# sevagh/demucs.cpp

Measured on AMD Instinct MI355X. Metric: audio-sec/s (xRT) htdemucs-4s 44.1kHz stereo, ~4-min track with overlap-add (BASELINE configs[2]), higher is better.
Workload: dtype f32 (exact bf16x3 operand split, fp32 accumulate)

## Files before the change

demucs_cpp_amd/binding.py:

```python
from __future__ import annotations

import ctypes
import os
from typing import List, Optional, Tuple

import numpy as np

ROOT = os.path.dirname(os.path.dirname(os.path.abspath(__file__)))
LIB_PATH = os.environ.get("DMX_LIB", os.path.join(ROOT, "demucs_cpp_amd", "lib", "libdemucs_hip.so"))

LAYOUT_EIGEN = 0
LAYOUT_PLANAR = 1
SEGMENT_SAMPLES = 343980
MAX_SHIFT = 22050
MAX_BAG = 8

EXPORTS = [
    "dmx_last_error", "dmx_device_count", "dmx_model_load", "dmx_model_free", "dmx_model_n_sources",
    "dmx_model_n_tensors", "dmx_model_device", "dmx_ctx_create", "dmx_ctx_free", "dmx_ctx_segment_samples",
    "dmx_ctx_max_batch", "dmx_ctx_arena_bytes", "dmx_ctx_synchronize", "dmx_ctx_set_stream", "dmx_segment_infer",
    "dmx_segment_infer_device", "dmx_track_infer", "dmx_track_geometry", "dmx_track_stats_device",
    "dmx_track_gather_device", "dmx_track_overlap_add_device", "dmx_debug_tap", "dmx_debug_n_ops",
    "dmx_debug_profile", "dmx_ctx_set_model", "dmx_model_clone",
    "dmx_debug_plan_info", "dmx_debug_op_info", "dmx_debug_arena_fill", "dmx_debug_arena_io", "dmx_debug_run_op", "dmx_debug_op_cfgs",
# ... 104 lines not shown
        L.dmx_remix_two_stems.argtypes = [ci, ci, ci, vp, vp]
        L.dmx_remix_check.argtypes = [ci, vp]
        L.dmx_tracks_infer_remix.argtypes = [vp, vp, ci, vp, ci, vp, vp, ci, ctypes.c_float, vp, vp, vp, vp, ci, vp, vp]
        L.dmx_remix_encode_device.argtypes = [ci, vp, ci, i64, i64, vp, vp, vp, vp, vp]
        L.dmx_remix_encode.argtypes = [ci, vp, ci, i64, vp, vp, vp, vp]
        L.dmx_flac_bound.argtypes = [ci, i64]
        L.dmx_flac_bound.restype = i64
        L.dmx_flac_workspace_bytes.argtypes = [ci, i64]
        L.dmx_flac_workspace_bytes.restype = i64
        L.dmx_flac_encode_device.argtypes = [ci, vp, ci, i64, ci, vp, vp, vp, vp]
        L.dmx_flac_encode.argtypes = [ci, vp, ci, i64, ci, vp, vp]
        L.dmx_tracks_infer_flac.argtypes = [vp, vp, ci, vp, ci, vp, vp, ci, ctypes.c_float, vp, vp, ci, vp, vp, vp, ci, vp, vp]
        L.dmx_track_geometry.argtypes = [vp, i64, ci, ctypes.POINTER(i64), ctypes.POINTER(ci), ctypes.POINTER(i64)]
        L.dmx_track_stats_device.argtypes = [vp, fp, i64, fp]
        L.dmx_track_gather_device.argtypes = [vp, fp, i64, fp, ci, vp, ci, fp]
        L.dmx_track_overlap_add_device.argtypes = [vp, fp, ci, i64, ci, fp, fp, ci]
        L.dmx_debug_tap.argtypes = [vp, ctypes.c_char_p, vp, fp]
        L.dmx_debug_n_ops.argtypes = [vp]
        L.dmx_debug_profile.argtypes = [vp, ci, ci, ctypes.c_char_p, ci]
        L.dmx_debug_plan_info.argtypes = [vp, ci, vp, vp, vp, vp]
        L.dmx_debug_op_info.argtypes = [vp, ci, ci, ctypes.c_char_p, ci]
        L.dmx_debug_arena_fill.argtypes = [vp, ci, ctypes.c_uint]
        L.dmx_debug_arena_io.argtypes = [vp, i64, i64, fp, ci]
        L.dmx_debug_run_op.argtypes = [vp, ci, ci]
        L.dmx_debug_op_cfgs.argtypes = [vp, ci, ci, vp, ci]
        L.dmx_debug_run_op_as.argtypes = [vp, ci, ci, ci, ci, ctypes.c_char_p, ci]
        L.dmx_ctx_set_model.argtypes = [vp, vp]
        L.dmx_engine_create.argtypes = [ctypes.POINTER(ctypes.c_char_p), ci, ctypes.POINTER(ci), ci, ci, ci, ctypes.POINTER(vp)]
        L.dmx_engine_free.argtypes = [vp]
        L.dmx_engine_set_finish.argtypes = [vp, ci]
        for f in ("dmx_engine_n_devices", "dmx_engine_n_models", "dmx_engine_n_sources", "dmx_engine_transport", "dmx_engine_finish"):
            getattr(L, f).argtypes = [vp]
        L.dmx_engine_root_ctx.argtypes = [vp, ci]
        L.dmx_engine_root_ctx.restype = vp
        L.dmx_engine_track_infer.argtypes = [vp, fp, i64, ctypes.POINTER(ci), fp, ci, vp, vp]
        _lib = L
    return _lib


def _chk(rc):
    if rc != 0:
        raise DmxError(rc, lib().dmx_last_error().decode(errors="replace"))


DEBUG_NO_KERNEL = 6


def parse_op_info(text: str) -> dict:
    d = {}
    for word in text.split():
        k, _, v = word.partition("=")
        if k in ("reads", "writes", "scratch", "rowstat"):
            d[k] = [tuple(int(x) for x in r.split(":")) for r in v.split(",") if r]
        elif k in ("name", "label"):
            d[k] = v
        else:
            d[k] = int(v)
    return d


def device_count() -> int:
    return lib().dmx_device_count()


class Model:

    def __init__(self, path: str, device: int = 0):
        self.h = ctypes.c_void_p()
        _chk(lib().dmx_model_load(path.encode(), device, ctypes.byref(self.h)))
        self.n_sources = lib().dmx_model_n_sources(self.h)
        self.n_tensors = lib().dmx_model_n_tensors(self.h)
        self.arch = lib().dmx_model_arch(self.h)
        self.device = device

    def close(self):
        if self.h:
            lib().dmx_model_free(self.h)
            self.h = ctypes.c_void_p()

    def __del__(self):
        try:
            self.close()
        except Exception:
            pass


def default_gemm() -> int:
    return lib().dmx_default_gemm()


def set_default_gemm(gemm: int):
    _chk(lib().dmx_set_default_gemm(gemm))


def split_weights(w: np.ndarray):
    w = np.ascontiguousarray(w, np.float32).ravel()
    w1 = np.zeros(w.size, np.uint16)
    w2 = np.zeros(w.size, np.uint16)
    bad = lib().dmx_debug_split_weights(w.ctypes.data, w.size, w1.ctypes.data, w2.ctypes.data)
    return w1, w2, int(bad)


def split_activations(x: np.ndarray, device: int = 0) -> np.ndarray:
    x = np.ascontiguousarray(x, np.float32).ravel()
    planes = np.zeros((3, x.size), np.uint16)
    _chk(lib().dmx_debug_split_activations(device, x.ctypes.data, x.size, planes.ctypes.data))
    return planes
# ... 574 lines not shown
```

demucs_cpp_amd/csrc/api.cpp:

```cpp
#include "api_internal.h"
#include "tracks_plan.h"
#include "plan_describe.h"

#include <algorithm>
#include <atomic>
#include <cstdarg>
#include <cstdio>
#include <cstdlib>
#include <cmath>
#include <cstring>
#include <cctype>
#include <cerrno>
#include <climits>
#include <fcntl.h>
#include <pthread.h>
#include <signal.h>
#include <sys/mman.h>
#include <sys/stat.h>
#include <unistd.h>

using namespace dmx;

static thread_local std::string g_err;
int dmx_fail(int code, const char *fmt, ...)
// ... 245 lines not shown
            (void)hipFree(m->dWh);
    }
    delete m;
}
extern "C" int dmx_model_n_sources(const dmx_model *m) { return m ? m->pm.n_sources : 0; }
extern "C" int dmx_model_n_tensors(const dmx_model *m) { return m ? m->pm.n_tensors : 0; }
extern "C" int dmx_model_device(const dmx_model *m) { return m ? m->device : -1; }
extern "C" int dmx_model_arch(const dmx_model *m) { return m ? m->pm.arch : 0; }

static bool validate_gemm(const Op &op, std::string &why)
{
    const IGemm &g = op.g;
    const bool al = ((i64)g.L0 * g.Cin) % 4 == 0 && (g.stride0 * g.Cin) % 4 == 0 && (g.pad0 * g.Cin) % 4 == 0 &&
                    g.seg0 % 4 == 0 && g.K % 4 == 0 && g.xBatchStride % 4 == 0 && (g.S1 == 1 || g.seg0 % 16 == 0) &&
                    (g.cfg == kDirectCfg || (g.Cin % 4 == 0 && g.seg0 % g.Cin == 0 && g.S1 * (g.seg0 / g.Cin) <= 31));
    if (g.epi == EPI_KPL || g.epi == EPI_VT)
    {
        if (g.choice.arith == 0)
        {
            why = "op " + op.name + ": K / V plane projection without its exact-split kernel";
            return false;
        }
        return true;
    }
    GemmArgs k{};
    fill_gemm_geometry(k, g);
    const bool exists = (g.cfg == kDirectCfg ? launch_dgemm(k, nullptr, true) : launch_igemm(g.cfg, k, nullptr, true)) == 0;
    if (!al || !exists)
    {
        why = "op " + op.name + (al ? ": no kernel instantiated for its (tile, prologue, epilogue)" : ": staging alignment contract violated");
        return false;
    }
    return true;
}
static bool validate_plan(const Plan &p, std::string &why)
{
    for (const Op &op : p.ops)
        if (op.kind == OP_IGEMM && !validate_gemm(op, why))
            return false;
    return true;
}

static Plan *get_plan(dmx_ctx *c, int batch)
{
    auto it = c->plans.find(batch);
    if (it != c->plans.end())
        return it->second.get();
    auto p = std::make_unique<Plan>();
    const bool planesOff = getenv("DMX_KV_PLANES") && atoi(getenv("DMX_KV_PLANES")) == 0;
    AttnArgs kv{};
    kv.hs = c->m->pm.dim / 8;
    const bool kvPlanes = c->gemm != DMX_GEMM_F32 && !planesOff && c->m->pm.arch != 3 && launch_attention_split(kv, nullptr, true) == 0;
    build_chosen_plan(c->m->pm, c->seg, batch, c->gemm, kvPlanes, model_facts(c->m), split_lin_mode(), *p);
    for (Op &op : p->ops)
        if (op.kind == OP_ATTENTION)
        {
            AttnArgs t{};
            t.hs = op.at.hs;
            op.at.split = c->gemm != DMX_GEMM_F32 && launch_attention_split(t, nullptr, true) == 0 ? 1 : 0;
        }
    Plan *raw = p.get();
    c->plans[batch] = std::move(p);
    return raw;
}

struct SharedLane
{
    static const int kSlots = 64;
    std::atomic<int> ready;
    std::atomic<int> pid[kSlots];
    pthread_mutex_t mu;
};
struct LstmLane
{
    std::mutex mu;
    hipEvent_t ev = nullptr;
    bool recorded = false;
    SharedLane *shared = nullptr;
};
static std::mutex g_lanesMu;
static std::vector<std::unique_ptr<LstmLane>> g_lanes;
static std::vector<SharedLane *> g_sharedRegistered;

static bool pid_alive(int pid) { return pid > 0 && (kill((pid_t)pid, 0) == 0 || errno != ESRCH); }

static int shared_lane_peers(SharedLane *sl)
{
    const int self = (int)getpid();
    int n = 0;
    for (int i = 0; i < SharedLane::kSlots; ++i)
    {
        int p = sl->pid[i].load(std::memory_order_acquire);
        if (p == 0 || p == self)
            continue;
        if (pid_alive(p))
            ++n;
        else
            sl->pid[i].compare_exchange_strong(p, 0);
    }
    return n;
}

static SharedLane *open_shared_lane(int device)
{
    if (const char *e = getenv("DMX_LSTM_SHARED_LANE"))
        if (atoi(e) == 0)
            return nullptr;
    auto give_up = [](const char *what) -> SharedLane * {
        fprintf(stderr, "demucs_hip: the process-shared LSTM lane is unavailable (%s: %s); several Demucs v3 processes on one GPU are not ordered\n", what,
                strerror(errno));
        return nullptr;
    };
// ... 406 lines not shown
            k.Wb2 = c->m->dWb + c->m->blobFloats + 512 + g.w_w;
            rc = launch_igemm_split(g.choice, g.cfg, k, s);
            break;
        }
        if (rc != 0)
            return fail(DMX_ERR_ARG, "internal error: the kernel chosen for op %s does not exist (%s: family %d, cfg %d pro %d epi %d)", op.name.c_str(),
                        g.choice.label ? g.choice.label : "none", g.choice.family, g.cfg, g.pro, g.epi);
        break;
    }
    case OP_DCONV_ROW:
    {
        const DconvRow &r = op.dr;
        DconvRowArgs k{};
        k.x = a(r.x), k.B = r.B, k.T = r.T, k.F = r.F, k.C = r.C, k.hid = r.hid, k.eps = r.eps, k.zero = A + zeroOff;
        k.img[0] = w(r.img_w[0]), k.img[1] = w(r.img_w[1]);
        if (launch_dconv_row(k, s) != 0)
            return fail(DMX_ERR_ARG, "internal error: no row-resident DConv kernel for op %s (C %d hidden %d T %d)", op.name.c_str(), r.C, r.hid, r.T);
        break;
    }
    case OP_STATS_REDUCE:
    {
        const StatsReduce &r = op.sr;
        launch_stats_reduce(ReduceArgs{a(r.rowstat), a(r.out), r.B, r.R, r.NB, r.G0, r.count, r.mode, r.eps,
                                       reinterpret_cast<double *>(a(r.scratch)), r.nchunk},
                            s);
        break;
    }
    case OP_STFT:
    {
        const Stft &t = op.stft;
        launch_stft(StftArgs{a(t.mix), a(t.x), a(t.rowstat), a(t.rowstatT), t.B, t.T, t.seg, t.pad, a(t.window), a(t.twiddle)}, s);
        break;
    }
    case OP_LAYERNORM:
    {
        const LayerNorm &l = op.ln;
        launch_layernorm(LnArgs{a(l.x), a(l.y), l.rows, l.D, l.rowsPerBatch, w(l.w_w), w(l.b_w), a(l.pe), l.eps}, s);
        break;
    }
    case OP_GN_APPLY:
    {
        const GnApply &g = op.gn;
        launch_gn_apply(GnArgs{a(g.x), a(g.y), a(g.res), g.B, g.rows, g.C, a(g.stats), w(g.w_w), w(g.b_w)}, s);
        break;
    }
    case OP_ATTENTION:
    {
        const Attention &t = op.at;
        AttnArgs k{a(t.q), a(t.k), a(t.v), a(t.o), t.ldq, t.ldk, t.ldv, t.ldo, t.qBatch, t.kBatch, t.vBatch,
                   t.oBatch, t.B, t.Tq, t.Tk, t.H, t.hs, t.scale};
        k.kpl = t.kpl >= 0 ? reinterpret_cast<const unsigned short *>(A + t.kpl) : nullptr;
        k.vt = t.vt >= 0 ? reinterpret_cast<const unsigned short *>(A + t.vt) : nullptr;
        k.kvPlane = (i64)t.B * t.Tk * t.H * t.hs;
        if (!(t.split && launch_attention_split(k, s) == 0))
        {
            if (t.kpl >= 0)
                return fail(DMX_ERR_ARG, "internal error: attention op %s reads operand planes but has no exact-split kernel", op.name.c_str());
            launch_attention(k, s);
        }
        break;
    }
    case OP_ISTFT:
    {
        const Istft &t = op.istft;
        if (!(t.fused && c->fuseIstft))
            launch_istft(IstftArgs{a(t.x), a(t.stats), a(t.frames), t.B, t.T, t.S, a(t.window), a(t.twiddle)}, s);
        break;
    }
    case OP_OLA:
    {
        const Ola &o = op.ola;
        if (o.x >= 0 && c->fuseIstft)
            launch_istft_ola(IstftOlaArgs{a(o.x), a(o.stats), a(o.xt), a(o.statsT), a(o.wss), a(o.window), a(o.twiddle), a(o.out), o.B, o.T,
                                          o.S, o.seg, o.pad, 0, 0, a(o.rden)},
                             s);
        else
            launch_ola(OlaArgs{a(o.frames), a(o.xt), a(o.statsT), a(o.wss), a(o.out), o.B, o.T, o.S, o.seg, o.pad}, s);
        break;
    }
    case OP_GROUP_STATS:
    {
        const GroupStats &g = op.gs;
        launch_group_stats(GroupStatsArgs{a(g.x), a(g.out), reinterpret_cast<double *>(a(g.scratch)), g.B, g.rows, g.C, g.G, g.eps}, s);
        break;
    }
    case OP_GN_ACT:
    {
        const GnAct &g = op.ga;
        launch_gn_act(GnActArgs{a(g.x), a(g.y), a(g.stats), a(g.res), w(g.w_w), w(g.b_w), w(g.scale_w), g.B, g.rowsIn, g.C, g.G, g.mode,
                                g.rowOff, g.rowsOut},
                      s);
        break;
    }
    case OP_LSTM:
    {
        const Lstm &l = op.lstm;
        LstmLane *lane = c->capturing ? nullptr : lstm_lane(c->m->device);
        std::unique_lock<std::mutex> laneLock;
        if (lane)
        {
            laneLock = std::unique_lock<std::mutex>(lane->mu);
            if (!lane->ev)
                HIPCHK(hipEventCreateWithFlags(&lane->ev, hipEventDisableTiming));
            if (lane->recorded)
                HIPCHK(hipStreamWaitEvent(s, lane->ev, 0));
        }
// ... 1681 lines not shown
```

demucs_cpp_amd/csrc/attention_common.h:

```cpp
#pragma once
#include "kernels.h"

namespace dmx
{

typedef float f32x4 __attribute__((ext_vector_type(4)));

__device__ __forceinline__ float max3f(float a, float b, float c) { return __builtin_fmaxf(__builtin_fmaxf(a, b), c); }
static constexpr float kDeferLog2 = 16.0f;
static constexpr float kLog2e = 1.44269504088896340736f;

__device__ __forceinline__ float quad_lanes_max(float x)
{
    typedef unsigned u32x2 __attribute__((ext_vector_type(2)));
    u32x2 r = __builtin_amdgcn_permlane16_swap(__float_as_uint(x), __float_as_uint(x), false, false);
    x = fmaxf(__uint_as_float(r[0]), __uint_as_float(r[1]));
    r = __builtin_amdgcn_permlane32_swap(__float_as_uint(x), __float_as_uint(x), false, false);
    return fmaxf(__uint_as_float(r[0]), __uint_as_float(r[1]));
}
__device__ __forceinline__ float quad_lanes_sum(float x)
{
    typedef unsigned u32x2 __attribute__((ext_vector_type(2)));
    u32x2 r = __builtin_amdgcn_permlane16_swap(__float_as_uint(x), __float_as_uint(x), false, false);
    x = __uint_as_float(r[0]) + __uint_as_float(r[1]);
    r = __builtin_amdgcn_permlane32_swap(__float_as_uint(x), __float_as_uint(x), false, false);
    return __uint_as_float(r[0]) + __uint_as_float(r[1]);
}

template <int DF, bool MASK, bool LOC>
__device__ __forceinline__ void att_softmax_pre(f32x4 (&sT)[4], f32x4 (&o)[DF], float &mrun, float &lrun, float &mcur, int t, int h4, int Tk,
                                                int qrow, float gq)
{
    constexpr int KT = 64;
    if constexpr (LOC)
    {
#pragma unroll
        for (int kf = 0; kf < 4; ++kf)
#pragma unroll
            for (int r = 0; r < 4; ++r)
            {
                const int key = t * KT + 16 * kf + 4 * h4 + r;
                const float dist = fabsf((float)(key - qrow));
                sT[kf][r] = key == qrow ? -100.0f * kLog2e : sT[kf][r] - dist * gq;
            }
    }
    if constexpr (MASK)
    {
#pragma unroll
        for (int kf = 0; kf < 4; ++kf)
#pragma unroll
            for (int r = 0; r < 4; ++r)
                if (t * KT + 16 * kf + 4 * h4 + r >= Tk)
                    sT[kf][r] = -INFINITY;
// ... 4 lines not shown
    tmx2 = max3f(tmx2, sT[2][0], sT[2][1]);
    float tmx3 = max3f(sT[2][2], sT[2][3], sT[3][0]);
    tmx3 = max3f(tmx3, sT[3][1], sT[3][2]);
    tmax = max3f(tmax, tmx2, fmaxf(tmx3, sT[3][3]));
    tmax = quad_lanes_max(tmax);
    float mnew = mrun;
    if (__builtin_amdgcn_ballot_w64(tmax > mnew + kDeferLog2) != 0ull)
    {
        mnew = fmaxf(mnew, tmax);
        const float alpha = __builtin_amdgcn_exp2f(mrun - mnew);
        lrun *= alpha;
        mrun = mnew;
#pragma unroll
        for (int d = 0; d < DF; ++d)
        {
            o[d][0] *= alpha;
            o[d][1] *= alpha;
            o[d][2] *= alpha;
            o[d][3] *= alpha;
        }
    }
    mcur = mnew;
}
__device__ __forceinline__ void att_softmax_post(f32x4 (&sT)[4], float &lrun, float mcur)
{
    float ps[4] = {0.f, 0.f, 0.f, 0.f};
#pragma unroll
    for (int kf = 0; kf < 4; ++kf)
#pragma unroll
        for (int r = 0; r < 4; ++r)
        {
            const float pv = __builtin_amdgcn_exp2f(sT[kf][r] - mcur);
            sT[kf][r] = pv;
            ps[kf] += pv;
        }
    lrun += (ps[0] + ps[1]) + (ps[2] + ps[3]);
}

__device__ __forceinline__ bool att_tile_of_block(const AttnArgs &p, unsigned &qt, unsigned &bh)
{
    if (p.xcdMap)
    {
        const unsigned xcd = blockIdx.x & 7u, j = blockIdx.x >> 3;
        const unsigned g = j / p.nQt;
        qt = j - g * p.nQt;
        bh = g * 8u + xcd;
        return bh < (unsigned)(p.B * p.H);
    }
    bh = blockIdx.x / p.nQt;
    qt = blockIdx.x - bh * p.nQt;
    return true;
}

inline bool att_use_big_shape(const AttnArgs &a)
{
    const long wg128 = (long)((a.Tq + 127) / 128) * a.H * a.B, wg64 = (long)((a.Tq + 63) / 64) * a.H * a.B;
    const double costBig = (double)((wg128 + 511) / 512), costSmall = 0.6 * (double)((wg64 + 511) / 512);
    return wg128 >= 1024 && costBig <= costSmall;
}

}
```

demucs_cpp_amd/csrc/attention_split.hip:

```cpp
#include "attention_common.h"
#include "igemm_common.h"
#include <cstdlib>
#include <type_traits>

namespace dmx
{

__device__ __forceinline__ int swzK(int key) { return (key >> 1) & 7; }
__device__ __forceinline__ int swzV(int dim) { return ((dim >> 1) & 1) | (((dim >> 3) & 1) << 1) | (((dim >> 2) & 1) << 2); }

template <int HS, int QF, bool PL>
__global__ __launch_bounds__(256, 2) void attention_split_kernel(const AttnArgs p)
{
    constexpr int DF = HS / 16;
    constexpr int KT = 64;
    constexpr int NS = 8;
    constexpr int KSL = HS / 8;
    constexpr int KCH = (KT * KSL + 255) / 256;
    constexpr int DQ = HS / 4;
    static_assert(HS == 64 || HS == 48, "head dims of htdemucs (512 / 8, 384 / 8)");

    __shared__ u32x4 Kp0[3][KT][NS], Kp1[3][KT][NS];
    __shared__ u32x4 Vp[3][HS][NS];

    const int tid = threadIdx.x, lane = tid & 63, wave = tid >> 6;
    const int l15 = lane & 15, h4 = lane >> 4;
    unsigned qt, bh;
    if (!att_tile_of_block(p, qt, bh))
        return;
    const int b = (int)(bh / (unsigned)p.H), head = (int)(bh - (unsigned)b * (unsigned)p.H);
    const int q0 = (int)qt * (64 * QF) + wave * (16 * QF);
    const float *Q = p.q + (i64)b * p.qB + head * HS;
    const float *K = p.k + (i64)b * p.kB + head * HS;
    const float *V = p.v + (i64)b * p.vB + head * HS;

    if constexpr (KSL < NS)
    {
        for (int i = tid; i < 2 * 3 * KT * (NS - KSL); i += 256)
        {
            const int sl = KSL + i % (NS - KSL), key = (i / (NS - KSL)) % KT, pl = (i / ((NS - KSL) * KT)) % 3, bf = i / ((NS - KSL) * KT * 3);
            (bf ? Kp1 : Kp0)[pl][key][sl ^ swzK(key)] = u32x4{0u, 0u, 0u, 0u};
        }
    }

    const float qs = p.scale * kLog2e;
    u32x4 qp[3][QF][2];
#pragma unroll
    for (int f = 0; f < QF; ++f)
    {
        const int qr = min(q0 + 16 * f + l15, p.Tq - 1);
#pragma unroll
        for (int kk = 0; kk < 2; ++kk)
        {
            const int d0 = 32 * kk + 8 * h4;
            f32x4 v0 = f32x4{0.f, 0.f, 0.f, 0.f}, v1 = v0;
            if (d0 < HS)
            {
                v0 = *reinterpret_cast<const f32x4 *>(Q + (i64)qr * p.ldq + d0);
                v1 = *reinterpret_cast<const f32x4 *>(Q + (i64)qr * p.ldq + d0 + 4);
            }
            unsigned h1[4], h2[4], h3[4];
            split3_pk(v0[0] * qs, v0[1] * qs, h1[0], h2[0], h3[0]);
            split3_pk(v0[2] * qs, v0[3] * qs, h1[1], h2[1], h3[1]);
            split3_pk(v1[0] * qs, v1[1] * qs, h1[2], h2[2], h3[2]);
            split3_pk(v1[2] * qs, v1[3] * qs, h1[3], h2[3], h3[3]);
            qp[0][f][kk] = u32x4{h1[0], h1[1], h1[2], h1[3]};
            qp[1][f][kk] = u32x4{h2[0], h2[1], h2[2], h2[3]};
            qp[2][f][kk] = u32x4{h3[0], h3[1], h3[2], h3[3]};
        }
    }

    f32x4 kreg[KCH][2], vreg[4];
    const int vh4 = tid & 3, vhalf = (tid >> 2) & 1, vdq = ((tid >> 3) & 1) + 2 * ((tid >> 4) & 7), vs = tid >> 7;
    const int vkq4 = 8 * vs + 4 * vhalf + vh4;
    const bool vOk = vdq < DQ;
    auto load_k = [&](int t0) {
#pragma unroll
        for (int i = 0; i < KCH; ++i)
        {
            const int c = min(tid + 256 * i, KT * KSL - 1);
            const int key = c / KSL, sl = c - key * KSL;
            const i64 r = min(t0 + key, p.Tk - 1);
            kreg[i][0] = *reinterpret_cast<const f32x4 *>(K + r * p.ldk + 8 * sl);
            kreg[i][1] = *reinterpret_cast<const f32x4 *>(K + r * p.ldk + 8 * sl + 4);
        }
    };
    auto load_v = [&](int t0) {
#pragma unroll
        for (int j = 0; j < 4; ++j)
        {
            const i64 r = min(t0 + 4 * vkq4 + j, p.Tk - 1);
            vreg[j] = *reinterpret_cast<const f32x4 *>(V + r * p.ldv + 4 * (vOk ? vdq : 0));
        }
    };
    auto store_k = [&](int buf) {
#pragma unroll
        for (int i = 0; i < KCH; ++i)
        {
            const int c = tid + 256 * i;
            if (KT * KSL % 256 != 0 && c >= KT * KSL)
                continue;
            const int key = c / KSL, sl = c - key * KSL;
            unsigned h1[4], h2[4], h3[4];
            split3_pk(kreg[i][0][0], kreg[i][0][1], h1[0], h2[0], h3[0]);
            split3_pk(kreg[i][0][2], kreg[i][0][3], h1[1], h2[1], h3[1]);
            split3_pk(kreg[i][1][0], kreg[i][1][1], h1[2], h2[2], h3[2]);
            split3_pk(kreg[i][1][2], kreg[i][1][3], h1[3], h2[3], h3[3]);
            u32x4(*Kp)[KT][NS] = buf ? Kp1 : Kp0;
            const int sw = sl ^ swzK(key);
            Kp[0][key][sw] = u32x4{h1[0], h1[1], h1[2], h1[3]};
            Kp[1][key][sw] = u32x4{h2[0], h2[1], h2[2], h2[3]};
            Kp[2][key][sw] = u32x4{h3[0], h3[1], h3[2], h3[3]};
        }
    };
    auto store_v = [&]() {
        if (!vOk)
            return;
#pragma unroll
        for (int c = 0; c < 4; ++c)
        {
            unsigned a1, a2, a3, b1, b2, b3;
            split3_pk(vreg[0][c], vreg[1][c], a1, a2, a3);
            split3_pk(vreg[2][c], vreg[3][c], b1, b2, b3);
            const int dim = 4 * vdq + c;
            const int sw = (4 * vs + vh4) ^ swzV(dim);
            *(reinterpret_cast<u32x2 *>(&Vp[0][dim][sw]) + vhalf) = u32x2{a1, b1};
            *(reinterpret_cast<u32x2 *>(&Vp[1][dim][sw]) + vhalf) = u32x2{a2, b2};
            *(reinterpret_cast<u32x2 *>(&Vp[2][dim][sw]) + vhalf) = u32x2{a3, b3};
        }
    };

    const int drow = lane >> 3, dpos = lane & 7;
    const int D = p.H * HS;
    const int wv = __builtin_amdgcn_readfirstlane(wave);
    auto dma_k = [&](int t0, int buf) {
        u32x4(*Kp)[KT][NS] = buf ? Kp1 : Kp0;
#pragma unroll
        for (int pl = 0; pl < 3; ++pl)
#pragma unroll
            for (int i = 0; i < 2; ++i)
            {
                const int c = 2 * wv + i, key = 8 * c + drow;
                const int src = dpos ^ swzK(key);
                const i64 r = (i64)b * p.Tk + min(t0 + key, p.Tk - 1);
                const unsigned short *g = p.kpl + (i64)pl * p.kvPlane + r * D + head * HS + 8 * src;
                if (KSL == NS || src < KSL)
                    load_to_lds_b128(reinterpret_cast<const float *>(g), reinterpret_cast<float4 *>(&Kp[pl][8 * c][0]));
            }
    };
    auto dma_v = [&](int t) {
        const int nt = p.Tk >> 6;
        const i64 tile = ((i64)b * p.H + head) * nt + min(t, nt - 1);
#pragma unroll
        for (int pl = 0; pl < 3; ++pl)
#pragma unroll
            for (int i = 0; i < 2; ++i)
            {
                const int c = wv + 4 * i;
                if (c < HS / 8)
                {
                    const int dim = 8 * c + drow;
                    const unsigned short *g = p.vt + (i64)pl * p.kvPlane + (tile * HS + dim) * 64 + 8 * (dpos ^ swzV(dim));
                    load_to_lds_b128(reinterpret_cast<const float *>(g), reinterpret_cast<float4 *>(&Vp[pl][8 * c][0]));
                }
            }
    };

    f32x4 o[QF][DF];
    float mrun[QF], lrun[QF], mcur[QF];
#pragma unroll
    for (int f = 0; f < QF; ++f)
    {
        mrun[f] = -INFINITY;
        lrun[f] = 0.f;
        mcur[f] = 0.f;
#pragma unroll
        for (int d = 0; d < DF; ++d)
            o[f][d] = f32x4{0.f, 0.f, 0.f, 0.f};
    }

    const int ksw = swzK(l15), vsw = swzV(l15);

    auto scores = [&](int buf, f32x4 (*sT)[4]) {
        u32x4(*Kp)[KT][NS] = buf ? Kp1 : Kp0;
#pragma unroll
        for (int f = 0; f < QF; ++f)
#pragma unroll
            for (int kf = 0; kf < 4; ++kf)
                sT[f][kf] = f32x4{0.f, 0.f, 0.f, 0.f};
#pragma unroll
        for (int kk = 0; kk < 2; ++kk)
#pragma unroll
            for (int kf0 = 0; kf0 < 4; kf0 += 2)
            {
                bf16x8 ka[2][3];
#pragma unroll
                for (int u = 0; u < 2; ++u)
#pragma unroll
                    for (int pl = 0; pl < 3; ++pl)
                        ka[u][pl] = __builtin_bit_cast(bf16x8, Kp[pl][16 * (kf0 + u) + l15][(4 * kk + h4) ^ ksw]);
                constexpr int TA[6] = {2, 0, 1, 1, 0, 0}, TB[6] = {0, 2, 1, 0, 1, 0};
#pragma unroll
                for (int tm = 0; tm < 6; ++tm)
#pragma unroll
                    for (int u = 0; u < 2; ++u)
#pragma unroll
                        for (int f = 0; f < QF; ++f)
                            sT[f][kf0 + u] = __builtin_amdgcn_mfma_f32_16x16x32_bf16(ka[u][TA[tm]], __builtin_bit_cast(bf16x8, qp[TB[tm]][f][kk]),
                                                                                      sT[f][kf0 + u], 0, 0, 0);
            }
    };
    auto pvprod = [&](f32x4 (*sT)[4]) {
#pragma unroll
        for (int s = 0; s < 2; ++s)
        {
            bf16x8 pp[QF][3];
#pragma unroll
            for (int f = 0; f < QF; ++f)
            {
                unsigned h1[4], h2[4], h3[4];
                split3_pk(sT[f][2 * s][0], sT[f][2 * s][1], h1[0], h2[0], h3[0]);
                split3_pk(sT[f][2 * s][2], sT[f][2 * s][3], h1[1], h2[1], h3[1]);
                split3_pk(sT[f][2 * s + 1][0], sT[f][2 * s + 1][1], h1[2], h2[2], h3[2]);
                split3_pk(sT[f][2 * s + 1][2], sT[f][2 * s + 1][3], h1[3], h2[3], h3[3]);
                pp[f][0] = __builtin_bit_cast(bf16x8, u32x4{h1[0], h1[1], h1[2], h1[3]});
                pp[f][1] = __builtin_bit_cast(bf16x8, u32x4{h2[0], h2[1], h2[2], h2[3]});
                pp[f][2] = __builtin_bit_cast(bf16x8, u32x4{h3[0], h3[1], h3[2], h3[3]});
            }
#pragma unroll
            for (int d0 = 0; d0 < DF; d0 += 2)
            {
                constexpr int ND = 2;
                bf16x8 va[ND][3];
#pragma unroll
                for (int u = 0; u < ND; ++u)
                    if (d0 + u < DF)
#pragma unroll
                        for (int pl = 0; pl < 3; ++pl)
                            va[u][pl] = __builtin_bit_cast(bf16x8, Vp[pl][16 * (d0 + u) + l15][(4 * s + h4) ^ vsw]);
                constexpr int TA[6] = {2, 0, 1, 1, 0, 0}, TB[6] = {0, 2, 1, 0, 1, 0};
#pragma unroll
                for (int tm = 0; tm < 6; ++tm)
#pragma unroll
                    for (int u = 0; u < ND; ++u)
                        if (d0 + u < DF)
#pragma unroll
                            for (int f = 0; f < QF; ++f)
                                o[f][d0 + u] = __builtin_amdgcn_mfma_f32_16x16x32_bf16(va[u][TA[tm]], pp[f][TB[tm]], o[f][d0 + u], 0, 0, 0);
            }
        }
    };

    const int nt = (p.Tk + KT - 1) / KT;
    const bool partial = (p.Tk % KT) != 0;
    if constexpr (PL)
    {
        dma_k(0, 0);
        asm volatile("s_waitcnt vmcnt(0)" ::: "memory");
        __syncthreads();
        auto tilep = [&](int t, auto parTag) {
            constexpr int PAR = decltype(parTag)::value;
            dma_v(t);
            __builtin_amdgcn_sched_barrier(0);
            dma_k((t + 1) * KT, PAR ^ 1);
            f32x4 sT[QF][4];
            scores(PAR, sT);
#pragma unroll
            for (int f = 0; f < QF; ++f)
            {
                att_softmax_pre<DF, false, false>(sT[f], o[f], mrun[f], lrun[f], mcur[f], t, h4, p.Tk, 0, 0.f);
                att_softmax_post(sT[f], lrun[f], mcur[f]);
            }
            asm volatile("s_waitcnt vmcnt(6)" ::: "memory");
            __syncthreads();
            pvprod(sT);
            asm volatile("s_waitcnt vmcnt(0)" ::: "memory");
            __syncthreads();
        };
        int t = 0;
        for (; t + 1 < nt; t += 2)
        {
            tilep(t, std::integral_constant<int, 0>{});
            tilep(t + 1, std::integral_constant<int, 1>{});
        }
        if (t < nt)
            tilep(t, std::integral_constant<int, 0>{});
    }
    else
    {
    load_k(0);
    load_v(0);
    store_k(0);
    load_k(KT);
    __syncthreads();
    auto tile = [&](int t, auto parTag, auto maskTag) {
        constexpr int PAR = decltype(parTag)::value;
        constexpr bool MASK = decltype(maskTag)::value;
        store_v();
        load_v((t + 1) * KT);
        f32x4 sT[QF][4];
        scores(PAR, sT);
#pragma unroll
        for (int f = 0; f < QF; ++f)
        {
            att_softmax_pre<DF, MASK, false>(sT[f], o[f], mrun[f], lrun[f], mcur[f], t, h4, p.Tk, 0, 0.f);
            att_softmax_post(sT[f], lrun[f], mcur[f]);
        }
        __syncthreads();
        pvprod(sT);
        store_k(PAR ^ 1);
        load_k((t + 2) * KT);
        __syncthreads();
    };
    const std::integral_constant<int, 0> even{};
    const std::integral_constant<int, 1> odd{};
    int t = 0;
    for (; t + 2 < nt; t += 2)
    {
        tile(t, even, std::false_type{});
        tile(t + 1, odd, std::false_type{});
    }
    if (t + 1 < nt)
    {
        tile(t, even, std::false_type{});
        if (partial)
            tile(t + 1, odd, std::true_type{});
        else
            tile(t + 1, odd, std::false_type{});
    }
    else if (partial)
        tile(t, even, std::true_type{});
    else
        tile(t, even, std::false_type{});
    }

#pragma unroll
    for (int f = 0; f < QF; ++f)
    {
        const float l = quad_lanes_sum(lrun[f]);
        const float inv = 1.0f / l;
        const int qr = q0 + 16 * f + l15;
        if (qr < p.Tq)
        {
            float *O = p.o + (i64)b * p.oB + (i64)qr * p.ldo + head * HS;
#pragma unroll
            for (int d = 0; d < DF; ++d)
                *reinterpret_cast<float4 *>(O + 16 * d + 4 * h4) =
                    make_float4(o[f][d][0] * inv, o[f][d][1] * inv, o[f][d][2] * inv, o[f][d][3] * inv);
        }
    }
}

int launch_attention_split(const AttnArgs &a0, hipStream_t s, bool dry)
{
    if (a0.hs != 64 && a0.hs != 48)
        return -1;
    if (dry)
        return 0;
    constexpr int xcdMap = 1;
    AttnArgs a = a0;
    a.xcdMap = xcdMap;
    const bool big = att_use_big_shape(a);
    a.nQt = (unsigned)(big ? (a.Tq + 127) / 128 : (a.Tq + 63) / 64);
    const unsigned nbh = (unsigned)(a.B * a.H);
    const dim3 grid(xcdMap ? 8u * ((nbh + 7u) / 8u) * a.nQt : nbh * a.nQt);
    const bool planes = a.kpl && a.vt && a.Tk % 64 == 0;
#define DMX_ATT_LAUNCH(HS_, QF_)                                                                            \
    do                                                                                                      \
    {                                                                                                       \
        if (planes)                                                                                         \
            hipLaunchKernelGGL((attention_split_kernel<HS_, QF_, true>), grid, dim3(256), 0, s, a);          \
        else                                                                                                \
            hipLaunchKernelGGL((attention_split_kernel<HS_, QF_, false>), grid, dim3(256), 0, s, a);         \
    } while (0)
    if (big)
    {
        if (a.hs == 64)
            DMX_ATT_LAUNCH(64, 2);
        else
            DMX_ATT_LAUNCH(48, 2);
    }
    else
    {
        if (a.hs == 64)
            DMX_ATT_LAUNCH(64, 1);
        else
            DMX_ATT_LAUNCH(48, 1);
    }
#undef DMX_ATT_LAUNCH
    return 0;
}

}
```

demucs_cpp_amd/csrc/kernels.h:

```cpp
#pragma once
#include "gemm_select.h"
#include <hip/hip_runtime.h>
#include <cstdlib>

namespace dmx
{

struct FastDiv
{
    unsigned magic, shift;
};
inline FastDiv make_fastdiv(unsigned d)
{
    FastDiv f;
    f.magic = 0;
    f.shift = 0;
    if (d == 0)
        d = 1;
    if ((d & (d - 1)) == 0)
    {
        while ((1u << f.shift) < d)
            ++f.shift;
        return f;
    }
// ... 67 lines not shown
    int B, R, NB, G0;
    double count;
    int mode;
    float eps;
    double *scratch;
    int nchunk;
};
void launch_stats_reduce(const ReduceArgs &a, hipStream_t s);

struct StftArgs
{
    const float *mix;
    float *x, *rowstat, *rowstatT;
    int B, T, seg, pad;
    const float *window, *twiddle;
};
void launch_stft(const StftArgs &a, hipStream_t s);

struct LnArgs
{
    const float *x;
    float *y;
    int rows, D, rowsPerBatch;
    const float *w, *b, *pe;
    float eps;
};
void launch_layernorm(const LnArgs &a, hipStream_t s);

struct GnArgs
{
    const float *x;
    float *y;
    const float *res;
    int B, rows, C;
    const float *stats, *w, *b;
};
void launch_gn_apply(const GnArgs &a, hipStream_t s);

struct AttnArgs
{
    const float *q, *k, *v;
    float *o;
    int ldq, ldk, ldv, ldo;
    i64 qB, kB, vB, oB;
    int B, Tq, Tk, H, hs;
    float scale;
    unsigned nQt;
    int xcdMap;
    const float *decay;
    int ldd;
    i64 dB;
    const unsigned short *kpl, *vt;
    i64 kvPlane;
};

void launch_attention(const AttnArgs &a, hipStream_t s);
int launch_attention_split(const AttnArgs &a, hipStream_t s, bool dry = false);
int launch_attention_local(const AttnArgs &a, hipStream_t s);

struct IstftArgs
{
    const float *x, *stats;
    float *frames;
    int B, T, S;
    const float *window, *twiddle;
};
void launch_istft(const IstftArgs &a, hipStream_t s);

struct OlaArgs
{
    const float *frames, *xt, *statsT, *wss;
    float *out;
    int B, T, S, seg, pad;
};
void launch_ola(const OlaArgs &a, hipStream_t s);
struct IstftOlaArgs
{
    const float *x, *stats, *xt, *statsT, *wss, *window, *twiddle;
    float *out;
    int B, T, S, seg, pad;
    int nch, fpc;
    const float *rden;
};
void launch_istft_ola(const IstftOlaArgs &a, hipStream_t s);

struct GroupStatsArgs
{
    const float *x;
    float *out;
    double *partials;
    int B, rows, C, G;
    float eps;
};
void launch_group_stats(const GroupStatsArgs &a, hipStream_t s);
struct GnActArgs
{
    const float *x;
    float *y;
    const float *stats, *res, *w, *b, *scale;
    int B, rowsIn, C, G, mode, rowOff, rowsOut;
};
void launch_gn_act(const GnActArgs &a, hipStream_t s);
struct LstmArgs
{
    const float *xproj, *whh;
    float *out;
// ... 171 lines not shown
```

demucs_cpp_amd/csrc/plan.h:

```cpp
#pragma once
#include <cstdint>
#include <string>
#include <vector>

namespace dmx
{
typedef int64_t i64;
static inline int rup(int v, int m) { return (v + m - 1) / m * m; }

enum OpKind
{
    OP_IGEMM = 0,
    OP_STATS_REDUCE,
    OP_STFT,
    OP_LAYERNORM,
    OP_GN_APPLY,
    OP_ATTENTION,
    OP_ISTFT,
    OP_OLA,
    OP_TAP,
    OP_GROUP_STATS,
    OP_GN_ACT,
    OP_LSTM,
    OP_LOCAL_ATTN,
// ... 84 lines not shown
    int hterms = 0;
};

struct StatsReduce
{
    i64 rowstat;
    i64 out;
    int B, R;
    int NB;
    int G0;
    double count;
    int mode;
    float eps;
    i64 scratch;
    int nchunk;
};

struct Stft
{
    i64 mix;
    i64 x;
    i64 rowstat;
    i64 rowstatT;
    int B, T, seg, pad;
    i64 window, twiddle;
};

struct LayerNorm
{
    i64 x, y;
    int rows, D, rowsPerBatch;
    i64 w_w, b_w;
    i64 pe;
    float eps;
};

struct GnApply
{
    i64 x, y, res;
    int B, rows, C;
    i64 stats;
    i64 w_w, b_w;
};

struct Attention
{
    i64 q, k, v, o;
    int ldq, ldk, ldv, ldo;
    i64 qBatch, kBatch, vBatch, oBatch;
    int B, Tq, Tk, H, hs;
    float scale;
    int split;
    i64 kpl = -1, vt = -1;
};

struct Istft
{
    i64 x;
    i64 stats;
    i64 frames;
    int B, T, S;
    i64 window, twiddle;
    int fused;
};

struct Ola
{
    i64 frames;
    i64 xt;
    i64 statsT;
    i64 wss;
    i64 out;
    int B, T, S, seg, pad;
    i64 x, stats, window, twiddle;
    i64 rden;
};

struct GroupStats
{
    i64 x;
    i64 out;
    int B, rows, C, G;
    float eps;
    i64 scratch;
};
struct GnAct
{
    i64 x, y, stats, res;
    i64 w_w, b_w, scale_w;
    int B, rowsIn, C, G, mode, rowOff, rowsOut;
};
struct Lstm
{
    i64 xproj;
    i64 whh_w;
    i64 out;
    i64 sync;
    int B, T, H;
};
i64 lstm_sync_floats(int B, int H);
i64 lstm_xchg_floats(int B, int T, int H);
struct LocalAttn
{
    i64 qkvd;
    i64 out;
    int B, T, H, ld;
// ... 142 lines not shown
```

demucs_cpp_amd/csrc/plan_describe.h:

```cpp
#pragma once
#include "plan.h"
#include <algorithm>
#include <cstdio>
#include <string>

namespace dmx
{
inline std::string describe_choice(const IGemm &g)
{
    char t[256];
    snprintf(t, sizeof(t), "cfg=%d family=%d arith=%d wnf=%d label=%s BM=%d BN=%d NB=%d", g.cfg, g.choice.family, g.choice.arith, g.choice.wnf,
             g.choice.label ? g.choice.label : "-", kTileCfgs[g.cfg].BM, kTileCfgs[g.cfg].BN, g.NB);
    return t;
}

inline std::string describe_op(const Op &op)
{
    std::vector<Range> rd, wr, scr;
    op_access(op, rd, wr);
    if (op.kind == OP_STATS_REDUCE && op.sr.scratch >= 0)
        scr.push_back(Range{op.sr.scratch, op.sr.scratch + (i64)op.sr.B * op.sr.nchunk * 4});
    if (op.kind == OP_GROUP_STATS && op.gs.scratch >= 0)
        scr.push_back(Range{op.gs.scratch, op.gs.scratch + (i64)op.gs.B * op.gs.G * 32 * 4});
    if (op.kind == OP_LSTM && op.lstm.sync >= 0)
        scr.push_back(Range{op.lstm.sync, op.lstm.sync + lstm_xchg_floats(op.lstm.B, op.lstm.T, op.lstm.H)});
    std::string all = "name=" + op.name + " kind=" + std::to_string(op.kind) + " stream=" + std::to_string(op.stream);
    const std::vector<Range> *lists[3] = {&rd, &wr, &scr};
    const char *keys[3] = {" reads=", " writes=", " scratch="};
    for (int k = 0; k < 3; ++k)
    {
        all += keys[k];
        for (const Range &r : *lists[k])
            all += std::to_string(r.lo) + ":" + std::to_string(r.hi) + ",";
    }
    auto word = [&](const char *k, i64 v) { all += std::string(" ") + k + "=" + std::to_string(v); };
    switch (op.kind)
    {
    case OP_IGEMM:
    {
        const IGemm &g = op.g;
        const i64 M = (i64)g.B * g.P1 * g.P0;
        word("K", g.K), word("N", g.N), word("M", M), word("pro", g.pro), word("epi", g.epi), word("act", g.act), word("res", g.res >= 0);
        word("stat", g.rowstat >= 0), word("hterms", g.hterms);
        word("y", g.y), word("ldy", g.ldy), word("Kp", g.Kp), word("w_w", g.w_w), word("bias_w", g.bias_w), word("kvCol0", g.kvCol0);
        all += " " + describe_choice(g);
        if (g.rowstat >= 0)
            all += " rowstat=" + std::to_string(g.rowstat) + ":" + std::to_string(g.rowstat + M * std::max(g.NB, 1) * 2);
        if (g.kv >= 0)
            word("kv", g.kv), word("kvPlane", (i64)g.B * g.kvT * g.kvH * g.kvHs);
        break;
    }
    case OP_ATTENTION:
        all += std::string(" label=") + (op.at.split ? "attention_split" : "attention");
        word("K", op.at.hs), word("T", op.at.Tk), word("split", op.at.split), word("planes", op.at.kpl >= 0);
        if (op.at.kpl >= 0)
            word("kpl", op.at.kpl), word("vt", op.at.vt), word("kvPlane", (i64)op.at.B * op.at.Tk * op.at.H * op.at.hs);
        break;
    case OP_STATS_REDUCE: all += " label=stats_reduce", word("K", (i64)op.sr.R * op.sr.NB); break;
    case OP_STFT: all += " label=stft", word("K", 4096); break;
    case OP_LAYERNORM: all += " label=layernorm", word("K", op.ln.D); break;
    case OP_GN_APPLY: all += " label=gn_apply"; break;
    case OP_ISTFT: all += " label=istft", word("K", 4096), word("fused", op.istft.fused); break;
    case OP_OLA: all += op.ola.x >= 0 ? " label=istft_ola" : " label=ola", word("K", 4096), word("fused", op.ola.x >= 0); break;
    case OP_GROUP_STATS: all += " label=group_stats", word("K", (i64)op.gs.rows * (op.gs.C / op.gs.G)); break;
    case OP_GN_ACT: all += " label=gn_act", word("mode", op.ga.mode); break;
    case OP_LSTM: all += " label=lstm", word("K", op.lstm.H), word("T", op.lstm.T); break;
    case OP_LOCAL_ATTN: all += " label=local_attn", word("K", op.la.H / 4), word("T", op.la.T); break;
    case OP_DCONV_ROW: all += " label=dconv_row", word("K", 3 * op.dr.C), word("T", op.dr.T), word("H", op.dr.hid); break;
    default: all += " label=tap"; break;
    }
    return all;
}
}
```

Before: 3068.

## Add paired 512-thread attention kernel that ping-pongs two query tiles per workgroup

```diff
diff --git a/demucs_cpp_amd/binding.py b/demucs_cpp_amd/binding.py
--- a/demucs_cpp_amd/binding.py
+++ b/demucs_cpp_amd/binding.py
@@ -180,7 +180,7 @@
         k, _, v = word.partition("=")
         if k in ("reads", "writes", "scratch", "rowstat"):
             d[k] = [tuple(int(x) for x in r.split(":")) for r in v.split(",") if r]
-        elif k in ("name", "label"):
+        elif k in ("name", "label", "form"):
             d[k] = v
         else:
             d[k] = int(v)
diff --git a/demucs_cpp_amd/csrc/api.cpp b/demucs_cpp_amd/csrc/api.cpp
--- a/demucs_cpp_amd/csrc/api.cpp
+++ b/demucs_cpp_amd/csrc/api.cpp
@@ -321,12 +321,17 @@
     kv.hs = c->m->pm.dim / 8;
     const bool kvPlanes = c->gemm != DMX_GEMM_F32 && !planesOff && c->m->pm.arch != 3 && launch_attention_split(kv, nullptr, true) == 0;
     build_chosen_plan(c->m->pm, c->seg, batch, c->gemm, kvPlanes, model_facts(c->m), split_lin_mode(), *p);
+    const char *pairEnv = getenv("DMX_ATT_PAIR");
+    const int pairMode = !pairEnv ? 1 : atoi(pairEnv) == 0 ? 0 : atoi(pairEnv) == 2 ? 2 : 1;
     for (Op &op : p->ops)
         if (op.kind == OP_ATTENTION)
         {
-            AttnArgs t{};
-            t.hs = op.at.hs;
-            op.at.split = c->gemm != DMX_GEMM_F32 && launch_attention_split(t, nullptr, true) == 0 ? 1 : 0;
+            Attention &t = op.at;
+            AttnArgs k{};
+            k.hs = t.hs;
+            t.split = c->gemm != DMX_GEMM_F32 && launch_attention_split(k, nullptr, true) == 0 ? 1 : 0;
+            if (t.split)
+                t.form = att_select_form(t.Tq, t.Tk, t.H, t.B, t.hs, t.kpl >= 0 && t.vt >= 0, pairMode);
         }
     Plan *raw = p.get();
     c->plans[batch] = std::move(p);
@@ -839,6 +844,7 @@
         k.kpl = t.kpl >= 0 ? reinterpret_cast<const unsigned short *>(A + t.kpl) : nullptr;
         k.vt = t.vt >= 0 ? reinterpret_cast<const unsigned short *>(A + t.vt) : nullptr;
         k.kvPlane = (i64)t.B * t.Tk * t.H * t.hs;
+        k.form = t.form;
         if (!(t.split && launch_attention_split(k, s) == 0))
         {
             if (t.kpl >= 0)
diff --git a/demucs_cpp_amd/csrc/attention_common.h b/demucs_cpp_amd/csrc/attention_common.h
--- a/demucs_cpp_amd/csrc/attention_common.h
+++ b/demucs_cpp_amd/csrc/attention_common.h
@@ -1,4 +1,5 @@
 #pragma once
+#include "attention_select.h"
 #include "kernels.h"
 
 namespace dmx
@@ -109,11 +110,6 @@
     return true;
 }
 
-inline bool att_use_big_shape(const AttnArgs &a)
-{
-    const long wg128 = (long)((a.Tq + 127) / 128) * a.H * a.B, wg64 = (long)((a.Tq + 63) / 64) * a.H * a.B;
-    const double costBig = (double)((wg128 + 511) / 512), costSmall = 0.6 * (double)((wg64 + 511) / 512);
-    return wg128 >= 1024 && costBig <= costSmall;
-}
+inline bool att_use_big_shape(const AttnArgs &a) { return att_big_shape(a.Tq, a.H, a.B); }
 
 }
diff --git a/demucs_cpp_amd/csrc/attention_select.h b/demucs_cpp_amd/csrc/attention_select.h
--- /dev/null
+++ b/demucs_cpp_amd/csrc/attention_select.h
@@ -0,0 +1,47 @@
+#pragma once
+
+namespace dmx
+{
+
+enum AttentionForm
+{
+    ATT_FORM_WG64 = 0,
+    ATT_FORM_WG128 = 1,
+    ATT_FORM_PAIR = 2
+};
+inline const char *att_form_name(int form) { return form == ATT_FORM_PAIR ? "pair" : form == ATT_FORM_WG128 ? "wg128" : "wg64"; }
+
+inline bool att_big_shape(int Tq, int H, int B)
+{
+    const long wg128 = (long)((Tq + 127) / 128) * H * B, wg64 = (long)((Tq + 63) / 64) * H * B;
+    const double costBig = (double)((wg128 + 511) / 512), costSmall = 0.6 * (double)((wg64 + 511) / 512);
+    return wg128 >= 1024 && costBig <= costSmall;
+}
+
+inline bool att_pair_exists(int Tk, int hs, bool planes) { return planes && Tk > 0 && Tk % 64 == 0 && (hs == 64 || hs == 48); }
+
+static constexpr int kAttPairMinQTiles = 21;
+static constexpr long kAttPairMinTiles = 2016;
+
+inline int att_select_form(int Tq, int Tk, int H, int B, int hs, bool planes, int pairMode)
+{
+    const bool big = att_big_shape(Tq, H, B);
+    if (pairMode == 2 && att_pair_exists(Tk, hs, planes))
+        return ATT_FORM_PAIR;
+    const int qTiles = (Tq + 127) / 128;
+    if (pairMode == 1 && big && att_pair_exists(Tk, hs, planes) && qTiles >= kAttPairMinQTiles && (long)qTiles * H * B >= kAttPairMinTiles)
+        return ATT_FORM_PAIR;
+    return big ? ATT_FORM_WG128 : ATT_FORM_WG64;
+}
+
+constexpr int att_pair_barriers(int nt, int half) { return (half ? 1 : 0) + 2 + 2 * nt + (half ? 0 : 1); }
+constexpr bool att_pair_barriers_agree(int ntMax)
+{
+    for (int nt = 1; nt <= ntMax; ++nt)
+        if (att_pair_barriers(nt, 0) != att_pair_barriers(nt, 1))
+            return false;
+    return true;
+}
+static_assert(att_pair_barriers_agree(8), "the halves of a paired attention workgroup must pass the same number of barriers");
+
+}
diff --git a/demucs_cpp_amd/csrc/attention_split.hip b/demucs_cpp_amd/csrc/attention_split.hip
--- a/demucs_cpp_amd/csrc/attention_split.hip
+++ b/demucs_cpp_amd/csrc/attention_split.hip
@@ -9,9 +9,11 @@
 __device__ __forceinline__ int swzK(int key) { return (key >> 1) & 7; }
 __device__ __forceinline__ int swzV(int dim) { return ((dim >> 1) & 1) | (((dim >> 3) & 1) << 1) | (((dim >> 2) & 1) << 2); }
 
-template <int HS, int QF, bool PL>
-__global__ __launch_bounds__(256, 2) void attention_split_kernel(const AttnArgs p)
+template <int HS, int QF, bool PL, bool PAIR>
+__device__ __forceinline__ void attention_split_body(const AttnArgs &p, u32x4 (*Kp0)[64][8], u32x4 (*Kp1)[64][8], u32x4 (*Vp)[HS][8], const int tid,
+                                                     const unsigned qt, const unsigned bh, const int half, const bool live)
 {
+    static_assert(!PAIR || (PL && QF == 2), "the paired form exists for the 128-query planes kernel only");
     constexpr int DF = HS / 16;
     constexpr int KT = 64;
     constexpr int NS = 8;
@@ -20,14 +22,8 @@
     constexpr int DQ = HS / 4;
     static_assert(HS == 64 || HS == 48, "head dims of htdemucs (512 / 8, 384 / 8)");
 
-    __shared__ u32x4 Kp0[3][KT][NS], Kp1[3][KT][NS];
-    __shared__ u32x4 Vp[3][HS][NS];
-
-    const int tid = threadIdx.x, lane = tid & 63, wave = tid >> 6;
+    const int lane = tid & 63, wave = tid >> 6;
     const int l15 = lane & 15, h4 = lane >> 4;
-    unsigned qt, bh;
-    if (!att_tile_of_block(p, qt, bh))
-        return;
     const int b = (int)(bh / (unsigned)p.H), head = (int)(bh - (unsigned)b * (unsigned)p.H);
     const int q0 = (int)qt * (64 * QF) + wave * (16 * QF);
     const float *Q = p.q + (i64)b * p.qB + head * HS;
@@ -132,7 +128,7 @@
 
     const int drow = lane >> 3, dpos = lane & 7;
     const int D = p.H * HS;
-    const int wv = __builtin_amdgcn_readfirstlane(wave);
+    const int wv = __builtin_amdgcn_readfirstlane(wave) & 3;
     auto dma_k = [&](int t0, int buf) {
         u32x4(*Kp)[KT][NS] = buf ? Kp1 : Kp0;
 #pragma unroll
@@ -210,50 +206,119 @@
                                                                                       sT[f][kf0 + u], 0, 0, 0);
             }
     };
+    auto psplit = [&](int s, f32x4 (*sT)[4], bf16x8 (*pp)[3]) {
+#pragma unroll
+        for (int f = 0; f < QF; ++f)
+        {
+            unsigned h1[4], h2[4], h3[4];
+            split3_pk(sT[f][2 * s][0], sT[f][2 * s][1], h1[0], h2[0], h3[0]);
+            split3_pk(sT[f][2 * s][2], sT[f][2 * s][3], h1[1], h2[1], h3[1]);
+            split3_pk(sT[f][2 * s + 1][0], sT[f][2 * s + 1][1], h1[2], h2[2], h3[2]);
+            split3_pk(sT[f][2 * s + 1][2], sT[f][2 * s + 1][3], h1[3], h2[3], h3[3]);
+            pp[f][0] = __builtin_bit_cast(bf16x8, u32x4{h1[0], h1[1], h1[2], h1[3]});
+            pp[f][1] = __builtin_bit_cast(bf16x8, u32x4{h2[0], h2[1], h2[2], h2[3]});
+            pp[f][2] = __builtin_bit_cast(bf16x8, u32x4{h3[0], h3[1], h3[2], h3[3]});
+        }
+    };
+    auto pvmul = [&](int s, bf16x8 (*pp)[3]) {
+#pragma unroll
+        for (int d0 = 0; d0 < DF; d0 += 2)
+        {
+            constexpr int ND = 2;
+            bf16x8 va[ND][3];
+#pragma unroll
+            for (int u = 0; u < ND; ++u)
+                if (d0 + u < DF)
+#pragma unroll
+                    for (int pl = 0; pl < 3; ++pl)
+                        va[u][pl] = __builtin_bit_cast(bf16x8, Vp[pl][16 * (d0 + u) + l15][(4 * s + h4) ^ vsw]);
+            constexpr int TA[6] = {2, 0, 1, 1, 0, 0}, TB[6] = {0, 2, 1, 0, 1, 0};
+#pragma unroll
+            for (int tm = 0; tm < 6; ++tm)
+#pragma unroll
+                for (int u = 0; u < ND; ++u)
+                    if (d0 + u < DF)
+#pragma unroll
+                        for (int f = 0; f < QF; ++f)
+                            o[f][d0 + u] = __builtin_amdgcn_mfma_f32_16x16x32_bf16(va[u][TA[tm]], pp[f][TB[tm]], o[f][d0 + u], 0, 0, 0);
+        }
+    };
     auto pvprod = [&](f32x4 (*sT)[4]) {
 #pragma unroll
         for (int s = 0; s < 2; ++s)
         {
             bf16x8 pp[QF][3];
+            psplit(s, sT, pp);
+            pvmul(s, pp);
+        }
+    };
+
+    const int nt = (p.Tk + KT - 1) / KT;
+    const bool partial = (p.Tk % KT) != 0;
+    if constexpr (PAIR)
+    {
+        f32x4 sT[QF][4];
+        bf16x8 pp[2][QF][3];
+        const std::integral_constant<int, 0> even{};
+        const std::integral_constant<int, 1> odd{};
+        auto sync = [&]() {
+            __builtin_amdgcn_sched_barrier(0);
+            __syncthreads();
+            __builtin_amdgcn_sched_barrier(0);
+        };
+        auto alpha = [&](int t, auto parTag) {
+            constexpr int PAR = decltype(parTag)::value;
+            if (t >= 1)
+                dma_v(t);
+            __builtin_amdgcn_sched_barrier(0);
+            dma_k((t + 1) * KT, PAR ^ 1);
 #pragma unroll
             for (int f = 0; f < QF; ++f)
             {
-                unsigned h1[4], h2[4], h3[4];
-                split3_pk(sT[f][2 * s][0], sT[f][2 * s][1], h1[0], h2[0], h3[0]);
-                split3_pk(sT[f][2 * s][2], sT[f][2 * s][3], h1[1], h2[1], h3[1]);
-                split3_pk(sT[f][2 * s + 1][0], sT[f][2 * s + 1][1], h1[2], h2[2], h3[2]);
-                split3_pk(sT[f][2 * s + 1][2], sT[f][2 * s + 1][3], h1[3], h2[3], h3[3]);
-                pp[f][0] = __builtin_bit_cast(bf16x8, u32x4{h1[0], h1[1], h1[2], h1[3]});
-                pp[f][1] = __builtin_bit_cast(bf16x8, u32x4{h2[0], h2[1], h2[2], h2[3]});
-                pp[f][2] = __builtin_bit_cast(bf16x8, u32x4{h3[0], h3[1], h3[2], h3[3]});
+                att_softmax_pre<DF, false, false>(sT[f], o[f], mrun[f], lrun[f], mcur[f], t, h4, p.Tk, 0, 0.f);
+                att_softmax_post(sT[f], lrun[f], mcur[f]);
             }
-#pragma unroll
-            for (int d0 = 0; d0 < DF; d0 += 2)
-            {
-                constexpr int ND = 2;
-                bf16x8 va[ND][3];
-#pragma unroll
-                for (int u = 0; u < ND; ++u)
-                    if (d0 + u < DF)
-#pragma unroll
-                        for (int pl = 0; pl < 3; ++pl)
-                            va[u][pl] = __builtin_bit_cast(bf16x8, Vp[pl][16 * (d0 + u) + l15][(4 * s + h4) ^ vsw]);
-                constexpr int TA[6] = {2, 0, 1, 1, 0, 0}, TB[6] = {0, 2, 1, 0, 1, 0};
-#pragma unroll
-                for (int tm = 0; tm < 6; ++tm)
-#pragma unroll
-                    for (int u = 0; u < ND; ++u)
-                        if (d0 + u < DF)
-#pragma unroll
-                            for (int f = 0; f < QF; ++f)
-                                o[f][d0 + u] = __builtin_amdgcn_mfma_f32_16x16x32_bf16(va[u][TA[tm]], pp[f][TB[tm]], o[f][d0 + u], 0, 0, 0);
-            }
-        }
-    };
-
-    const int nt = (p.Tk + KT - 1) / KT;
-    const bool partial = (p.Tk % KT) != 0;
-    if constexpr (PL)
+            psplit(0, sT, pp[0]);
+            psplit(1, sT, pp[1]);
+            asm volatile("s_waitcnt vmcnt(0)" ::: "memory");
+            sync();
+        };
+        auto beta = [&](auto parTag, auto lastTag) {
+            constexpr int PAR = decltype(parTag)::value;
+            pvmul(0, pp[0]);
+            pvmul(1, pp[1]);
+            if constexpr (!decltype(lastTag)::value)
+                scores(PAR ^ 1, sT);
+            sync();
+        };
+        dma_k(0, 0);
+        __builtin_amdgcn_sched_barrier(0);
+        dma_v(0);
+        if (half)
+            sync();
+        asm volatile("s_waitcnt vmcnt(0)" ::: "memory");
+        sync();
+        scores(0, sT);
+        sync();
+        int t = 0;
+        for (; t + 2 < nt; t += 2)
+        {
+            alpha(t, even);
+            beta(even, std::false_type{});
+            alpha(t + 1, odd);
+            beta(odd, std::false_type{});
+        }
+        alpha(t, even);
+        if (t + 1 < nt)
+        {
+            beta(even, std::false_type{});
+            alpha(t + 1, odd);
+            beta(odd, std::true_type{});
+        }
+        else
+            beta(even, std::true_type{});
+    }
+    else if constexpr (PL)
     {
         dma_k(0, 0);
         asm volatile("s_waitcnt vmcnt(0)" ::: "memory");
@@ -340,7 +405,7 @@
         const float l = quad_lanes_sum(lrun[f]);
         const float inv = 1.0f / l;
         const int qr = q0 + 16 * f + l15;
-        if (qr < p.Tq)
+        if (live && qr < p.Tq)
         {
             float *O = p.o + (i64)b * p.oB + (i64)qr * p.ldo + head * HS;
 #pragma unroll
@@ -349,6 +414,43 @@
                     make_float4(o[f][d][0] * inv, o[f][d][1] * inv, o[f][d][2] * inv, o[f][d][3] * inv);
         }
     }
+    if constexpr (PAIR)
+        if (!half)
+        {
+            __builtin_amdgcn_sched_barrier(0);
+            __syncthreads();
+        }
+}
+
+template <int HS, int QF, bool PL>
+__global__ __launch_bounds__(256, 2) void attention_split_kernel(const AttnArgs p)
+{
+    __shared__ u32x4 Kp0[3][64][8], Kp1[3][64][8];
+    __shared__ u32x4 Vp[3][HS][8];
+    unsigned qt, bh;
+    if (!att_tile_of_block(p, qt, bh))
+        return;
+    attention_split_body<HS, QF, PL, false>(p, Kp0, Kp1, Vp, (int)threadIdx.x, qt, bh, 0, true);
+}
+
+template <int HS>
+__global__ __launch_bounds__(512, 1) void attention_split_pair_kernel(const AttnArgs p)
+{
+    __shared__ u32x4 Kp[2][2][3][64][8];
+    __shared__ u32x4 Vp[2][3][HS][8];
+    const int half = __builtin_amdgcn_readfirstlane((int)threadIdx.x >> 8);
+    const unsigned xcd = blockIdx.x & 7u, j0 = 2u * (blockIdx.x >> 3);
+    const unsigned nbh = (unsigned)(p.B * p.H);
+    if ((j0 / p.nQt) * 8u + xcd >= nbh)
+        return;
+    unsigned j = j0 + (unsigned)half;
+    const bool live = (j / p.nQt) * 8u + xcd < nbh;
+    if (!live)
+        j = j0;
+    const unsigned g = j / p.nQt;
+    if (half)
+        __builtin_amdgcn_s_setprio(1);
+    attention_split_body<HS, 2, true, true>(p, Kp[half][0], Kp[half][1], Vp[half], (int)threadIdx.x & 255, j - g * p.nQt, g * 8u + xcd, half, live);
 }
 
 int launch_attention_split(const AttnArgs &a0, hipStream_t s, bool dry)
@@ -360,11 +462,22 @@
     constexpr int xcdMap = 1;
     AttnArgs a = a0;
     a.xcdMap = xcdMap;
-    const bool big = att_use_big_shape(a);
+    const bool big = a.form != ATT_FORM_WG64;
     a.nQt = (unsigned)(big ? (a.Tq + 127) / 128 : (a.Tq + 63) / 64);
     const unsigned nbh = (unsigned)(a.B * a.H);
     const dim3 grid(xcdMap ? 8u * ((nbh + 7u) / 8u) * a.nQt : nbh * a.nQt);
     const bool planes = a.kpl && a.vt && a.Tk % 64 == 0;
+    if (a.form == ATT_FORM_PAIR)
+    {
+        if (!att_pair_exists(a.Tk, a.hs, planes))
+            return -1;
+        const dim3 pairs(8u * (((nbh + 7u) / 8u * a.nQt + 1u) / 2u));
+        if (a.hs == 64)
+            hipLaunchKernelGGL((attention_split_pair_kernel<64>), pairs, dim3(512), 0, s, a);
+        else
+            hipLaunchKernelGGL((attention_split_pair_kernel<48>), pairs, dim3(512), 0, s, a);
+        return 0;
+    }
 #define DMX_ATT_LAUNCH(HS_, QF_)                                                                            \
     do                                                                                                      \
     {                                                                                                       \
diff --git a/demucs_cpp_amd/csrc/kernels.h b/demucs_cpp_amd/csrc/kernels.h
--- a/demucs_cpp_amd/csrc/kernels.h
+++ b/demucs_cpp_amd/csrc/kernels.h
@@ -143,6 +143,7 @@
     i64 dB;
     const unsigned short *kpl, *vt;
     i64 kvPlane;
+    int form;
 };
 
 void launch_attention(const AttnArgs &a, hipStream_t s);
diff --git a/demucs_cpp_amd/csrc/plan.h b/demucs_cpp_amd/csrc/plan.h
--- a/demucs_cpp_amd/csrc/plan.h
+++ b/demucs_cpp_amd/csrc/plan.h
@@ -160,6 +160,7 @@
     float scale;
     int split;
     i64 kpl = -1, vt = -1;
+    int form = 0;
 };
 
 struct Istft
diff --git a/demucs_cpp_amd/csrc/plan_describe.h b/demucs_cpp_amd/csrc/plan_describe.h
--- a/demucs_cpp_amd/csrc/plan_describe.h
+++ b/demucs_cpp_amd/csrc/plan_describe.h
@@ -1,4 +1,5 @@
 #pragma once
+#include "attention_select.h"
 #include "plan.h"
 #include <algorithm>
 #include <cstdio>
@@ -53,6 +54,8 @@
     case OP_ATTENTION:
         all += std::string(" label=") + (op.at.split ? "attention_split" : "attention");
         word("K", op.at.hs), word("T", op.at.Tk), word("split", op.at.split), word("planes", op.at.kpl >= 0);
+        word("Tq", op.at.Tq), word("H", op.at.H), word("B", op.at.B);
+        all += std::string(" form=") + (op.at.split ? att_form_name(op.at.form) : "-");
         if (op.at.kpl >= 0)
             word("kpl", op.at.kpl), word("vt", op.at.vt), word("kvPlane", (i64)op.at.B * op.at.Tk * op.at.H * op.at.hs);
         break;
```

Result: faster. 3106 (median of 6 runs) (+1.2%).
